# aubin-tchoi/shot-fpfh

Hardware: AMD Instinct MI355X
Metric: descriptors/sec (SHOT+FPFH) on 1M-pt cloud (higher is better)
Workload: dtype f64

## Files before the change

shot_fpfh_amd/csrc/common.h:

```cpp
#pragma once
#include <hip/hip_runtime.h>

#include <cstdarg>
#include <cstdint>
#include <cstdio>
#include <cstring>
#include <map>
#include <atomic>
#include <tuple>
#include <string>
#include <vector>

#include "../../include/shotfpfh.h"

extern std::atomic<unsigned long long> g_sf_sync_count;
static inline hipError_t sf_counted_stream_sync(hipStream_t s)
{
    g_sf_sync_count.fetch_add(1, std::memory_order_relaxed);
    return hipStreamSynchronize(s);
}
#define hipStreamSynchronize(s) sf_counted_stream_sync(s)

#define SF_WAVE 64

// ... 82 lines not shown
    {
        const int rc = sf_palloc(ctx, out, count);
        if (rc == SF_OK) held.push_back((void *)*out);
        return rc;
    }
    void release(void *p)
    {
        for (auto &h : held)
            if (h == p) { sf_pool_release(ctx, p); h = nullptr; }
    }
    ~sf_pool_guard()
    {
        for (void *p : held)
            if (p) sf_pool_release(ctx, p);
    }
};

int sf_comm_allreduce_max_i32(sf_ctx *ctx, const int *send, int *recv, size_t n);
int sf_ctx_scratch(sf_ctx *ctx, size_t bytes, void **out);
#define SF_FLAG_ROWS_GATHER 1
#define SF_FLAG_VOXEL_ORDER 2
int sf_ctx_check_flag(sf_ctx *ctx);
#define SF_PINNED_BYTES 32768
int sf_ctx_pinned(sf_ctx *ctx, void **out);
hipEvent_t sf_ctx_event(sf_ctx *ctx);

struct sf_launch_timer {
    sf_ctx *ctx;
    const char *name;
    hipEvent_t e0 = nullptr, e1 = nullptr;
    bool active;
    sf_launch_timer(sf_ctx *c, const char *n)
        : ctx(c), name(n), active(c->profiling && (c->prof_only.empty() || c->prof_only == n))
    {
        if (active) {
            e0 = sf_ctx_event(ctx);
            e1 = sf_ctx_event(ctx);
            (void)hipEventRecord(e0, ctx->stream);
        }
    }
    ~sf_launch_timer()
    {
        if (active) {
            (void)hipEventRecord(e1, ctx->stream);
            sf_prof_entry &p = ctx->prof[name];
            p.launches++;
            p.pending.emplace_back(e0, e1);
        } else {
            ctx->prof[name].launches++;
        }
    }
};

#define SF_LAUNCH(ctx, name, kernel, grid, block, ...)                                   \
    do {                                                                                 \
        sf_launch_timer t_((ctx), (name));                                               \
        hipLaunchKernelGGL(kernel, (grid), (block), 0, (ctx)->stream, __VA_ARGS__);      \
    } while (0);                                                                         \
    SF_HIP(hipGetLastError())

struct sf_cloud {
    int64_t n = 0;
    double *xyz_orig = nullptr;
    double *nrm_orig = nullptr;
    int32_t *zperm = nullptr;
    int32_t *perm_int = nullptr;
    bool bbox_known = false;
    double bbox_lo[3] = {0, 0, 0}, bbox_hi[3] = {0, 0, 0};
    uint64_t grid_gen = 0;
    double cell = 0.0;
    double inv_cell = 0.0;
    double lo[3] = {0, 0, 0};
    int dim[3] = {1, 1, 1};
    int xsub = 1;
    int64_t ncell = 0;
    int32_t *cell_start = nullptr;
    int32_t *perm = nullptr;
    int32_t *inv_perm = nullptr;
    bool inv_perm_valid = false;
    double *xs = nullptr, *ys = nullptr, *zs = nullptr;
    double *rec = nullptr;
    bool normals_sorted = false;
    double nrm_max2 = -1.0;
    int64_t pop_begin = 0, pop_end = 0;
    double *z_orig = nullptr;
    std::vector<double> z_host;
    int32_t *cell_count = nullptr;
    int64_t cell_count_cap = 0;
    bool count_dirty = false;
    std::vector<int64_t> layer_first;
    std::map<std::pair<double, bool>, std::pair<double, int64_t>> list_stats;
    struct search_record {
        int64_t total = 0, n_overflow = 0, ovf_total = 0, cap = 0, hist[5] = {0, 0, 0, 0, 0};
        int32_t max_count = 0, max_count_all = 0;
        bool folded = false;
    };
    typedef std::tuple<double, double, int, int64_t, int64_t> search_key;
    std::map<search_key, search_record> search_records;
};

struct sf_nbrs {
    int64_t m = 0;
    double radius = 0.0;
    int64_t total = 0;
    int64_t max_count = 0;
    int64_t max_count_all = 0;
    bool view = false;
    bool self = false;
    int64_t self_begin = 0;
    double *qx = nullptr, *qy = nullptr, *qz = nullptr;
    int32_t *qrow = nullptr;
    int32_t *count = nullptr;
    int64_t *offset = nullptr;
    int32_t *idx = nullptr;
    int32_t *idx_ovf = nullptr;
    int64_t cap = 0;
    int64_t n_overflow = 0;
    int64_t hist[5] = {0, 0, 0, 0, 0};
    bool planned = false;
    int main_chunks = 4;
    int tail_limit = 0x7fffffff;
    int32_t *tail_sel = nullptr;
    int64_t n_tail = 0;
    int32_t *mid_sel = nullptr;
    int64_t n_mid = 0;
    int64_t view_first = 0;
    uint64_t grid_gen = 0;
};

static inline void sf_nbrs_stamp(sf_nbrs *nb, const sf_cloud *c) { nb->grid_gen = c->grid_gen; }
static inline int sf_nbrs_on_grid(const sf_nbrs *nb, const sf_cloud *c, const char *who)
{
    if (nb->grid_gen == c->grid_gen) return SF_OK;
    sf_set_error("%s: the neighbour lists were made on another grid of this cloud (build %llu, now %llu): a search with another "
                 "radius, a k-NN search or sf_cloud_build_grid rebuilt it -- search again, or use the lists before the next rebuild",
                 who, (unsigned long long)nb->grid_gen, (unsigned long long)c->grid_gen);
    return SF_ERR_STATE;
}

struct sf_spfh {
    int64_t n = 0;
    int64_t rows_alloc = 0;
    int n_bins = 0;
    int nb3 = 0;
    int stride = 0;
    int elem_bytes = 2;
    int bias = 0;
    int win_lo = 0;
    int win_len = 0;
    void *counts = nullptr;
    int32_t *k = nullptr;
    double *p4 = nullptr;
    unsigned *live = nullptr;
    uint8_t *packed = nullptr;
    uint8_t *hi = nullptr;
    unsigned host_live[2] = {0xffu, ~0u};
    bool host_live_valid = false;
    bool mask_known = false;
};

static inline int64_t sf_div_up(int64_t a, int64_t b) { return (a + b - 1) / b; }

struct sf_dispatch {
    int chunks = 4;
    int limit = 0x7fffffff;
    int tail_limit = 0x7fffffff;
    const int32_t *tail_sel = nullptr;
    int64_t n_tail = 0, view_first = 0;
    const int32_t *mid_sel = nullptr;
    int64_t n_mid = 0;
};
static inline sf_dispatch sf_nbrs_dispatch(const sf_nbrs *nb)
{
    sf_dispatch d;
    if (nb->planned) {
        d.chunks = nb->main_chunks;
        d.limit = nb->n_mid ? 64 * nb->main_chunks : nb->tail_limit;
        d.tail_limit = nb->tail_limit;
        d.tail_sel = nb->tail_sel;
        d.n_tail = nb->n_tail;
        d.mid_sel = nb->mid_sel;
        d.n_mid = nb->n_mid;
        d.view_first = nb->view_first;
    } else {
        const int64_t mx = nb->max_count > 0 ? nb->max_count : 1;
        d.chunks = mx <= 256 ? (int)sf_div_up(mx, 64) : 0;
    }
    return d;
}
```

shot_fpfh_amd/csrc/spfh.hip:

```cpp
#include <algorithm>
#include <cmath>
#include <cstring>

#include "common.h"
#include "device_util.h"

namespace {

#define SF_WIN_FPFH_BINS 11
struct fpfh_edges {
    double a[SF_WIN_FPFH_BINS + 1], p[SF_WIN_FPFH_BINS + 1], t[SF_WIN_FPFH_BINS + 1];
    double tan_t[SF_WIN_FPFH_BINS + 1];
    double p_inv_width;
};

__device__ inline int hist_bin(const double *e, int nb, double x)
{
    if (!(x >= e[0]) || x > e[nb]) return -1;
    int b = 0;
#pragma unroll
    for (int i = 1; i < SF_WIN_FPFH_BINS; ++i)
        if (i < nb && x >= e[i]) b = i;
    return b;
}

__device__ inline int theta_bin(const fpfh_edges &ed, int nb, double a, double b)
{
    const double band = 1e-13;
    const double aa = fabs(a);
    if (b > band * aa) {
        int bin = 0;
        double gap = 1.0e300;
#pragma unroll
        for (int i = 1; i < SF_WIN_FPFH_BINS; ++i)
            if (i < nb) {
                const double di = __builtin_fma(-ed.tan_t[i], b, a);
                bin += di >= 0.0 ? 1 : 0;
                gap = fmin(gap, fabs(di));
            }
        if (gap > band * (aa + fabs(ed.tan_t[1]) * b)) return bin;
    } else if (b < -band * aa) {
        return -1;
    }
    return hist_bin(ed.t, nb, atan2(a, b));
}

__device__ inline int theta_bin_fast(const fpfh_edges &ed, int nb, double a, double b, double E)
{
    const double band = 1e-13;
    const double aa = fabs(a) + E;
    if (b > band * aa) {
        int bin = 0;
        double gap = 1.0e300;
#pragma unroll
        for (int i = 1; i < SF_WIN_FPFH_BINS; ++i)
            if (i < nb) {
                const double di = __builtin_fma(-ed.tan_t[i], b, a);
                bin += di >= 0.0 ? 1 : 0;
                gap = fmin(gap, fabs(di));
            }
        return gap > band * (aa + fabs(ed.tan_t[1]) * b) + E ? bin : -2;
    }
    return b < -band * aa ? -1 : -2;
}

#ifndef SF_SPFH_WPB
#define SF_SPFH_WPB 2
#endif

template <typename CT, int NCH, int NB, bool SEL>
__global__ __launch_bounds__(64 * SF_SPFH_WPB) __attribute__((amdgpu_waves_per_eu((NCH == 0 || NCH >= 4) ? 5 : 6))) void k_spfh(const double *__restrict__ rec,
                                              const int64_t *__restrict__ offset, const int32_t *__restrict__ cnt,
    const int32_t *__restrict__ idx,
                                              int64_t m, int64_t self_begin, fpfh_edges ed, int nb_rt, int nb3, int stride,
                                              CT *__restrict__ counts, int32_t *__restrict__ kout, unsigned bias,
                                              double *__restrict__ p4, double mom_radius, double *__restrict__ cov,
                                              unsigned *__restrict__ live, int alpha_bin, double nrm_max,
                                              uint8_t *__restrict__ packed, int pack_b0, int pack_b1,
                                              uint8_t *__restrict__ hi, int limit, const int32_t *__restrict__ sel,
                                              int64_t nsel, int64_t view_first, int alpha_pair, int win_lo, int win_len)
{
    const int nb = NB > 0 ? NB : nb_rt;
    __shared__ unsigned int hist[SF_SPFH_WPB][SF_FAST_FPFH_BINS * SF_FAST_FPFH_BINS * SF_FAST_FPFH_BINS];
    const int lane = threadIdx.x & 63, wave = threadIdx.x >> 6;
    int64_t q = sf_uniform64(sf_xcd_block() * SF_SPFH_WPB + wave);
    if (SEL) {
        if (q >= nsel) return;
        q = (int64_t)sf_uniform(sel[q]) - view_first;
        if (q < 0) return;
    }
    if (q >= m) return;
    unsigned int *h = hist[wave];
    for (int b = lane; b < win_len; b += 64) h[b] = 0;
    const int64_t i = self_begin + q;
    const int64_t s = offset[q];
    const int k = cnt[q];
#ifndef SF_AB_NOLIMIT
    if (!SEL && sf_uniform(k) > limit) return;
#endif
    const double px = rec[6 * i + 0], py = rec[6 * i + 1], pz = rec[6 * i + 2];
    const double ux = rec[6 * i + 3], uy = rec[6 * i + 4], uz = rec[6 * i + 5];
    __builtin_amdgcn_wave_barrier();
    const double p_inv_width = ed.p_inv_width;
    const double uu = (ux * ux + uy * uy) + uz * uz;
    const double e_per_dist = 1.5e-14 * nrm_max * uu;
    auto pair = [&](double cx, double cy, double cz, double njx, double njy, double njz) {
        const double d2 = (cx * cx + cy * cy) + cz * cz;
        if (d2 > 0.0) {
            const double num = (cx * ux + cy * uy) + cz * uz;
            const double y0 = __builtin_amdgcn_rsq(d2);
            const double y1 = __builtin_fma(0.5 * y0, __builtin_fma(-(d2 * y0), y0, 1.0), y0);
            double phi = num * y1;
            const double pos = (phi - ed.p[0]) * p_inv_width;
            if (fabs(pos - rint(pos)) <= 1e-9) phi = num / sqrt(d2);
            const double b = (njx * ux + njy * uy) + __builtin_fma(njz, uz, 0.0);
            constexpr bool EVEN = NB > 0 && NB % 2 == 0;
            int ba = alpha_bin, bt = -2;
            if (alpha_bin >= 0 || (EVEN && alpha_pair >= 0)) {
                const double nc = (njx * cx + njy * cy) + njz * cz;
                bt = theta_bin_fast(ed, nb, nc * uu - b * num, b, e_per_dist * (d2 * y1) * 1.01);
            }
            if (!EVEN) {
                if (bt == -2) {
                    const double vx = cy * uz - cz * uy, vy = cz * ux - cx * uz, vz = cx * uy - cy * ux;
                    if (alpha_bin < 0) ba = hist_bin(ed.a, nb, (vx * njx + vz * njz) + vy * njy);
                    const double wx = uy * vz - uz * vy, wy = uz * vx - ux * vz, wz = ux * vy - uy * vx;
                    bt = theta_bin(ed, nb, (njx * wx + njz * wz) + njy * wy, b);
                }
            } else if (bt == -2 || alpha_bin < 0) {
                const double vx = cy * uz - cz * uy, vy = cz * ux - cx * uz, vz = cx * uy - cy * ux;
                if (bt == -2) {
                    const double wx = uy * vz - uz * vy, wy = uz * vx - ux * vz, wz = ux * vy - uy * vx;
                    bt = theta_bin(ed, nb, (njx * wx + njz * wz) + njy * wy, b);
                }
                if (alpha_bin < 0) {
                    const double alpha = (vx * njx + vz * njz) + vy * njy;
                    ba = alpha_pair >= 0 ? alpha_pair + (alpha >= ed.a[alpha_pair + 1] ? 1 : 0) : hist_bin(ed.a, nb, alpha);
                }
            }
            const int bp = hist_bin(ed.p, nb, phi);
            if ((ba | bp | bt) >= 0) atomicAdd(&h[(ba * nb + bp) * nb + bt - win_lo], 1u);
        }
    };
    double ws = 0, a11 = 0, a21 = 0, a31 = 0, a22 = 0, a32 = 0, a33 = 0;
    auto moments = [&](double cx, double cy, double cz) {
        const double w = mom_radius - sf_sqrt_fast((cx * cx + cy * cy) + cz * cz);
        ws += w;
        const double wx = cx * w, wy = cy * w, wz = cz * w;
        a11 = __builtin_fma(cx, wx, a11); a21 = __builtin_fma(cy, wx, a21); a31 = __builtin_fma(cz, wx, a31);
        a22 = __builtin_fma(cy, wy, a22); a32 = __builtin_fma(cz, wy, a32); a33 = __builtin_fma(cz, wz, a33);
    };
    if (NCH > 0) {
        constexpr int NC = NCH > 0 ? NCH : 1;
        const int ku = sf_uniform(k);
        int jj[NC];
#pragma unroll
        for (int c = 0; c < NC; ++c) {
            const int t = c * 64 + lane;
            jj[c] = -1;
            if (c == 0 || c * 64 < ku) jj[c] = t < k ? SF_LIST_LOAD(idx + s + t) : -1;
        }
        double cx[NC], cy[NC], cz[NC], ax[NC], ay[NC], az[NC];
#pragma unroll
        for (int c = 0; c < NC; ++c) {
            cx[c] = cy[c] = cz[c] = ax[c] = ay[c] = az[c] = 0.0;
            if (c == 0 || c * 64 < ku) {
                const int j = jj[c] < 0 ? 0 : jj[c];
                sf_load_pn(rec, j, cx[c], cy[c], cz[c], ax[c], ay[c], az[c]);
            }
        }
#pragma unroll
        for (int c = 0; c < NC; ++c)
            if ((c == 0 || c * 64 < ku) && jj[c] >= 0) {
                if (cov) moments(cx[c] - px, cy[c] - py, cz[c] - pz);
                pair(cx[c] - px, cy[c] - py, cz[c] - pz, ax[c], ay[c], az[c]);
            }
    } else {
        for (int t = lane; t < k; t += 64) {
            double x, y, z, a, b, c;
            sf_load_pn(rec, idx[s + t], x, y, z, a, b, c);
            if (cov) moments(x - px, y - py, z - pz);
            pair(x - px, y - py, z - pz, a, b, c);
        }
    }
    if (cov) {
        const double part[8] = {ws, a11, a21, a31, a22, a32, a33, 0.0};
        const double tot = sf_wave_sum8(part);
        const double wsum = __hiloint2double(__builtin_amdgcn_readlane(__double2hiint(tot), 0),
                                             __builtin_amdgcn_readlane(__double2loint(tot), 0));
        const double iw = sf_rcp_fast(wsum);
        const int e = lane >> 3;
        if ((lane & 7) == 0 && e >= 1 && e <= 6) cov[6 * q + e - 1] = tot * iw;
    }
    __builtin_amdgcn_wave_barrier();
    __threadfence_block();
    CT *row = counts + i * (int64_t)stride;
    bool hi_empty = false;
    if (live) {
        const unsigned v0 = lane < win_len ? h[lane] : 0u, v1 = lane + 64 < win_len ? h[lane + 64] : 0u;
        __builtin_nontemporal_store((CT)(v0 ^ bias), row + lane);
        __builtin_nontemporal_store((CT)(v1 ^ bias), row + lane + 64);
        if (hi && sf_uniform(k) > 255) {
            hi[i * 128 + lane] = (uint8_t)(v0 >> 8);
            hi[i * 128 + lane + 64] = (uint8_t)(v1 >> 8);
            hi_empty = __ballot(((v0 | v1) >> 8) != 0u) == 0ull;
        }
        if (packed && lane < 8) {
            const int first = 16 * (lane < 4 ? pack_b0 : pack_b1) + 4 * (lane & 3);
            unsigned w = 0u;
#pragma unroll
            for (int t = 0; t < 4; ++t) w |= (((first + t < win_len ? h[first + t] : 0u) ^ bias) & 0xffu) << (8 * t);
            reinterpret_cast<unsigned *>(packed + i * 32)[lane] = w;
        }
        const unsigned long long n0 = __ballot(v0 != 0u), n1 = __ballot(v1 != 0u);
        unsigned mask = 0u;
#pragma unroll
        for (int kq = 0; kq < 4; ++kq) {
            mask |= ((n0 >> (16 * kq)) & 0xffffull) ? 1u << kq : 0u;
            mask |= ((n1 >> (16 * kq)) & 0xffffull) ? 16u << kq : 0u;
        }
        if (lane == 0 && (mask & ~*live)) atomicOr(live, mask);
    } else {
        for (int b = lane; b < stride; b += 64) row[b] = (CT)((b < nb3 ? h[b] : 0u) ^ bias);
    }
    if (lane == 0) {
        kout[i] = k;
        if (p4) {
            double2 *o = reinterpret_cast<double2 *>(p4 + 4 * i);
            o[0] = make_double2(rec[6 * i + 0], rec[6 * i + 1]);
            o[1] = make_double2(rec[6 * i + 2], hi_empty ? -(double)k : (double)k);
        }
    }
}

__device__ inline void spfh_pack_row(const uint8_t *__restrict__ counts, uint8_t *__restrict__ packed, int64_t row, unsigned mask)
{
    const int b0 = mask ? __ffs(mask) - 1 : 0;
    const unsigned rest = mask & (mask - 1u);
    const int b1 = rest ? __ffs(rest) - 1 : (b0 + 1) & 7;
    const uint4 *src = reinterpret_cast<const uint4 *>(counts + row * 128);
    uint4 *dst = reinterpret_cast<uint4 *>(packed + row * 32);
    dst[0] = src[b0];
    dst[1] = src[b1];
}

__global__ __launch_bounds__(256) void k_spfh_pack(const uint8_t *__restrict__ counts, int64_t begin, int64_t end,
                                                   const unsigned *__restrict__ live, uint8_t *__restrict__ packed)
{
    const unsigned mask = live[0] & 0xffu;
    if (__popc(mask) > 2) return;
    const int64_t row = begin + (int64_t)blockIdx.x * blockDim.x + threadIdx.x;
    if (row < end) spfh_pack_row(counts, packed, row, mask);
}

__global__ __launch_bounds__(256) void k_spfh_repack(const uint8_t *__restrict__ counts, int64_t n, int64_t begin, int64_t end,
                                                     const unsigned *__restrict__ live, uint8_t *__restrict__ packed)
{
    const unsigned mask = live[0] & 0xffu, sig = live[1];
    if (__popc(mask) > 2 || sig == mask) return;
    for (int64_t row = (int64_t)blockIdx.x * blockDim.x + threadIdx.x; row < n; row += (int64_t)gridDim.x * blockDim.x)
        if (row < begin || row >= end) spfh_pack_row(counts, packed, row, mask);
}

__global__ void k_spfh_live_or(unsigned *__restrict__ live, unsigned det) { live[0] |= det; }

__global__ void k_spfh_pack_done(unsigned *__restrict__ live)
{
    const unsigned mask = live[0] & 0xffu;
    live[1] = __popc(mask) <= 2 ? mask : ~0u;
}

template <typename CT>
__global__ void k_spfh_export(const CT *__restrict__ counts, const int32_t *__restrict__ kk,
                              const int32_t *__restrict__ perm, int64_t n, int nb3, int stride, unsigned bias,
                              double *__restrict__ out, const uint8_t *__restrict__ hi, int win_lo, int win_len)
{
    int64_t g = (int64_t)blockIdx.x * blockDim.x + threadIdx.x;
    if (g >= n * nb3) return;
    int64_t i = g / nb3;
    int b = (int)(g - i * nb3);
    const int col = b - win_lo;
    unsigned cnt = 0u;
    if (col >= 0 && col < win_len) {
        cnt = (unsigned)counts[i * stride + col] ^ bias;
        if (hi && kk[i] > 255) cnt += 256u * (unsigned)hi[i * stride + col];
    }
    out[(int64_t)perm[i] * nb3 + b] = (double)cnt / (double)kk[i];
}

__device__ inline int hist_bin_search(const double *__restrict__ e, int nb, double x)
{
    if (!(x >= e[0]) || x > e[nb]) return -1;
    if (x == e[nb]) return nb - 1;
    int lo = 0, hi = nb + 1;
    while (lo < hi) {
        const int mid = (lo + hi) >> 1;
        if (e[mid] <= x) lo = mid + 1; else hi = mid;
    }
    return lo - 1;
}

__global__ __launch_bounds__(256) void k_spfh_generic(const double *__restrict__ rec, const int64_t *__restrict__ offset,
                                                      const int32_t *__restrict__ cnt, const int32_t *__restrict__ idx, int64_t m,
                                                      int64_t self_begin, const double *__restrict__ edges, int nb, int nb3,
                                                      int stride, unsigned *__restrict__ counts, int32_t *__restrict__ kk)
{
    const int lane = threadIdx.x & 63;
    const int64_t q = sf_uniform64(sf_xcd_block() * 4 + (threadIdx.x >> 6));
    if (q >= m) return;
    const int64_t i = self_begin + q, s = offset[q];
    const int k = cnt[q];
    unsigned *row = counts + i * (int64_t)stride;
    for (int b = lane; b < stride; b += 64) row[b] = 0u;
    if (lane == 0) kk[i] = k;
    __threadfence();
    double px, py, pz, ux, uy, uz;
    sf_load_pn(rec, (int)i, px, py, pz, ux, uy, uz);
    const double *ea = edges, *ep = edges + (nb + 1), *et = edges + 2 * (nb + 1);
    for (int t = lane; t < k; t += 64) {
        double x, y, z, nx, ny, nz;
        sf_load_pn(rec, idx[s + t], x, y, z, nx, ny, nz);
        const double cx = x - px, cy = y - py, cz = z - pz;
        const double dist = sqrt((cx * cx + cy * cy) + cz * cz);
        if (!(dist > 0.0)) continue;
        const double vx = cy * uz - cz * uy, vy = cz * ux - cx * uz, vz = cx * uy - cy * ux;
        const double wx = uy * vz - uz * vy, wy = uz * vx - ux * vz, wz = ux * vy - uy * vx;
        const double alpha = (vx * nx + vz * nz) + vy * ny;
        const double phi = (((cx * ux + cy * uy) + cz * uz) + 0.0) / dist;
        const double theta = atan2((nx * wx + nz * wz) + ny * wy, ((nx * ux + ny * uy) + nz * uz) + 0.0);
        const int ba = hist_bin_search(ea, nb, alpha), bp = hist_bin_search(ep, nb, phi), bt = hist_bin_search(et, nb, theta);
        if (ba < 0 || bp < 0 || bt < 0) continue;
        atomicAdd(&row[(ba * nb + bp) * nb + bt], 1u);
    }
}
}


static bool alpha_bins_within_reach(const double *edges_a, int nb, double reach, int *first, int *last)
{
    if (!(reach >= 0.0) || !std::isfinite(reach) || !(-reach > edges_a[0]) || !(reach < edges_a[nb])) return false;
    int lo = 0, hi = 0;
    for (int i = 1; i < nb; ++i) {
        if (edges_a[i] <= -reach) lo = i;
        if (edges_a[i] <= reach) hi = i;
    }
    *first = lo;
    *last = hi;
    return true;
}

static sf_spfh *spfh_create(sf_ctx *ctx, sf_cloud *c, int n_bins, int64_t max_count, double radius);

extern "C" sf_spfh *sf_spfh_create(sf_ctx *ctx, sf_cloud *c, int n_bins, int64_t max_count)
{
    return spfh_create(ctx, c, n_bins, max_count, 0.0);
}

extern "C" sf_spfh *sf_spfh_create_for_radius(sf_ctx *ctx, sf_cloud *c, int n_bins, int64_t max_count, double radius)
{
    return spfh_create(ctx, c, n_bins, max_count, radius);
}

extern "C" int sf_spfh_elem_bytes(const sf_spfh *sp) { return sp ? sp->elem_bytes : 0; }

static sf_spfh *spfh_create(sf_ctx *ctx, sf_cloud *c, int n_bins, int64_t max_count, double radius)
{
    if (!ctx || !c) { sf_set_error("sf_spfh_create: null argument"); return nullptr; }
    if (n_bins < 1 || n_bins > SF_MAX_FPFH_BINS) {
        sf_set_error("sf_spfh_create: n_bins=%d outside 1..%d (n_bins^3 bins per point)", n_bins, SF_MAX_FPFH_BINS);
        return nullptr;
    }
    if (hipSetDevice(ctx->device) != hipSuccess) { sf_set_error("hipSetDevice failed"); return nullptr; }
    sf_spfh *sp = new sf_spfh();
    sp->n = c->n;
    sp->n_bins = n_bins;
    sp->nb3 = n_bins * n_bins * n_bins;
    sp->win_lo = 0;
    sp->win_len = sp->nb3;
    bool window = false;
    if (sp->nb3 > 128 && n_bins <= SF_WIN_FPFH_BINS && max_count <= 65535 && radius > 0.0 && c->nrm_orig && !getenv("SF_FPFH_NO_WINDOW")) {
        double n2 = 0.0, ea[SF_WIN_FPFH_BINS + 1];
        if (sf_cloud_normals_max2(ctx, c, &n2) != SF_OK) { delete sp; return nullptr; }
        for (int i = 0; i <= n_bins; ++i) ea[i] = -1.0 + 2.0 * (double)i / (double)n_bins;
        int a0 = 0, a1 = 0;
        if (alpha_bins_within_reach(ea, n_bins, radius * n2 * (1.0 + 1e-6), &a0, &a1) && (a1 - a0 + 1) * n_bins * n_bins <= 128) {
            window = true;
            sp->win_lo = a0 * n_bins * n_bins;
            sp->win_len = (a1 - a0 + 1) * n_bins * n_bins;
        }
    }
    sp->elem_bytes = (max_count <= 65535 && (sp->nb3 <= 128 || window)) ? 1 : (max_count > 65535 ? 4 : 2);
    if (n_bins > SF_FAST_FPFH_BINS && !window) sp->elem_bytes = 4;
    sp->bias = sp->elem_bytes == 1 ? 128 : 0;
    sp->stride = 128;
    while (sp->stride < (window ? sp->win_len : sp->nb3)) sp->stride *= 2;
    if (n_bins > SF_FAST_FPFH_BINS && !window) sp->stride = (sp->nb3 + 3) & ~3;
    const int64_t nr = ctx->nranks > 0 ? ctx->nranks : 1;
    sp->rows_alloc = std::max<int64_t>(sf_div_up(c->n, nr) * nr, 1);
    size_t nn = (size_t)sp->rows_alloc;
    if ((double)nn * sp->stride * sp->elem_bytes > 2.0e11) {
        sf_set_error("sf_spfh_create: an SPFH table of %lld x %d bins does not fit the device", (long long)nn, sp->nb3);
        delete sp;
        return nullptr;
    }
    const bool bytes_tab = sp->elem_bytes == 1;
    bool ok = sf_pool_alloc(ctx, nn * sp->stride * sp->elem_bytes, &sp->counts) == SF_OK && sf_pool_alloc(ctx, nn * sizeof(int32_t), (void **)&sp->k) == SF_OK;
    if (ok && bytes_tab) ok = sf_pool_alloc(ctx, nn * 4 * sizeof(double), (void **)&sp->p4) == SF_OK;
    if (ok && bytes_tab && max_count > 255) ok = sf_pool_alloc(ctx, nn * 128, (void **)&sp->hi) == SF_OK;
    if (ok && bytes_tab)
        ok = sf_pool_alloc(ctx, 4 * sizeof(unsigned), (void **)&sp->live) == SF_OK && sf_pool_alloc(ctx, nn * 32, (void **)&sp->packed) == SF_OK &&
             hipMemsetAsync(sp->live, 0, 4 * sizeof(unsigned), ctx->stream) == hipSuccess &&
             hipMemsetAsync(sp->live, getenv("SF_FPFH_DENSE") ? 0xff : 0, sizeof(unsigned), ctx->stream) == hipSuccess &&
             hipMemsetAsync(sp->live + 1, 0xff, sizeof(unsigned), ctx->stream) == hipSuccess;
    if (!ok) {
        sf_set_error("sf_spfh_create: out of device memory");
        sf_spfh_free(ctx, sp);
        return nullptr;
    }
    sp->host_live[0] = getenv("SF_FPFH_DENSE") ? ~0u : 0u;
    sp->host_live[1] = ~0u;
    sp->host_live_valid = sp->mask_known = sp->elem_bytes == 1;
    return sp;
}

extern "C" void sf_spfh_free(sf_ctx *ctx, sf_spfh *sp)
{
    if (!sp) return;
    if (ctx) (void)hipStreamSynchronize(ctx->stream);
    for (void *p : {(void *)sp->counts, (void *)sp->k, (void *)sp->p4, (void *)sp->live, (void *)sp->packed, (void *)sp->hi})
        if (p) { if (ctx) sf_pool_release(ctx, p); else (void)hipFree(p); }
    delete sp;
}

static int spfh_compute(sf_ctx *ctx, sf_cloud *c, sf_nbrs *nb, sf_spfh *sp, const double *edges, double *cov)
{
    if (!ctx || !c || !nb || !sp || !edges) { sf_set_error("sf_spfh_compute: null argument"); return SF_ERR_ARG; }
    if (!nb->self) { sf_set_error("sf_spfh_compute: needs a sf_radius_search_self result"); return SF_ERR_ARG; }
    SF_CHECK(sf_nbrs_on_grid(nb, c, "sf_spfh_compute"));
    if (sp->n != c->n || nb->self_begin + nb->m > sp->n) { sf_set_error("sf_spfh_compute: table/cloud size mismatch"); return SF_ERR_ARG; }
    if (sp->elem_bytes == 1 && nb->max_count > 255 && !sp->hi) {
        sf_set_error("sf_spfh_compute: neighbourhood of %lld points needs a wider table (pass max_count to sf_spfh_create)",
                     (long long)nb->max_count);
        return SF_ERR_ARG;
    }
    if (sp->elem_bytes <= 2 && nb->max_count > 65535) {
        sf_set_error("sf_spfh_compute: neighbourhood of %lld points needs a 32-bit table (pass max_count to sf_spfh_create)",
                     (long long)nb->max_count);
        return SF_ERR_ARG;
    }
    SF_HIP(hipSetDevice(ctx->device));
    SF_CHECK(sf_cloud_ensure_sorted_normals(ctx, c));
    if (sp->n_bins > SF_FAST_FPFH_BINS && sp->elem_bytes != 1) {
        if (cov) { sf_set_error("sf_spfh_compute_moments: n_bins=%d has no shared-sweep form (use sf_spfh_compute)", sp->n_bins); return SF_ERR_UNSUPPORTED; }
        const int64_t mg = nb->m;
        if (!mg) return SF_OK;
        sf_pool_guard tmp(ctx);
        double *dedges = nullptr;
        const size_t ne = (size_t)3 * (sp->n_bins + 1);
        SF_CHECK(tmp.alloc(&dedges, ne));
        SF_HIP(hipMemcpyAsync(dedges, edges, ne * sizeof(double), hipMemcpyHostToDevice, ctx->stream));
        SF_LAUNCH(ctx, "k6_spfh", k_spfh_generic, dim3(sf_xcd_grid(sf_div_up(mg, 4))), dim3(256), c->rec, nb->offset, nb->count,
                  nb->idx, mg, nb->self_begin, (const double *)dedges, sp->n_bins, sp->nb3, sp->stride, (unsigned *)sp->counts, sp->k);
        SF_HIP(hipStreamSynchronize(ctx->stream));
        return SF_OK;
    }
    fpfh_edges ed;
    const int nbn = sp->n_bins;
    for (int i = 0; i <= SF_WIN_FPFH_BINS; ++i) {
        ed.a[i] = edges[i <= nbn ? i : nbn];
        ed.p[i] = edges[(nbn + 1) + (i <= nbn ? i : nbn)];
        ed.t[i] = edges[2 * (nbn + 1) + (i <= nbn ? i : nbn)];
        ed.tan_t[i] = std::tan(ed.t[i]);
    }
    ed.p_inv_width = (double)nbn / (ed.p[nbn] - ed.p[0]);
    const int64_t m = nb->m;
    if (!m) return SF_OK;
    int alpha_bin = -1, alpha_pair = -1;
    double nrm_max = 1.0;
    {
        double n2 = 0.0;
        SF_CHECK(sf_cloud_normals_max2(ctx, c, &n2));
        nrm_max = std::sqrt(n2) * (1.0 + 1e-12);
        const double reach = nb->radius * n2 * (1.0 + 1e-9);
        double nearest = INFINITY;
        for (int i = 0; i <= nbn; ++i) nearest = std::min(nearest, std::fabs(ed.a[i]));
        if (std::isfinite(reach) && reach < nearest)
            for (int i = 0; i < nbn; ++i)
                if (ed.a[i] < 0.0 && 0.0 < ed.a[i + 1]) alpha_bin = i;
        int a0 = 0, a1 = 0;
        const bool within = alpha_bins_within_reach(ed.a, nbn, reach, &a0, &a1);
        if (alpha_bin < 0 && within && a1 == a0 + 1) alpha_pair = a0;
        if (getenv("SF_FPFH_NO_ALPHA_SHORTCUT")) alpha_bin = alpha_pair = -1;
        if (sp->elem_bytes == 1 && sp->win_len != sp->nb3) {
            if (!within || a0 * nbn * nbn < sp->win_lo || (a1 + 1) * nbn * nbn > sp->win_lo + sp->win_len) {
                sf_set_error("sf_spfh_compute: the table keeps bins %d .. %d of %d (created for a smaller radius); a search radius of %g "
                             "reaches other alpha bins -- create the table for this radius", sp->win_lo, sp->win_lo + sp->win_len - 1,
                             sp->nb3, nb->radius);
                return SF_ERR_STATE;
            }
        }
    }
    const dim3 grid(sf_xcd_grid(sf_div_up(m, SF_SPFH_WPB))), block(64 * SF_SPFH_WPB);
    const sf_dispatch dsp = sf_nbrs_dispatch(nb);
    const dim3 grid_tail(sf_xcd_grid(sf_div_up(dsp.n_tail > 0 ? dsp.n_tail : 1, SF_SPFH_WPB)));
    const dim3 grid_mid(sf_xcd_grid(sf_div_up(dsp.n_mid > 0 ? dsp.n_mid : 1, SF_SPFH_WPB)));
    uint8_t *const hi_rows = sp->elem_bytes == 1 ? sp->hi : nullptr;
#define SF_SPFH_NB(NAME, GRID, CT, NCH, NB, SEL, SELP, NSEL)                                                            \
    SF_LAUNCH(ctx, NAME, (k_spfh<CT, NCH, NB, SEL>), GRID, block, c->rec, nb->offset, nb->count, nb->idx, m,            \
              nb->self_begin, ed, nbn, sp->nb3, sp->stride, (CT *)sp->counts, sp->k, (unsigned)sp->bias, sp->p4, nb->radius, cov, \
              sizeof(CT) == 1 ? sp->live : (unsigned *)nullptr, alpha_bin, nrm_max, fused_packed, fused_b0, fused_b1,   \
              hi_rows, dsp.limit, SELP, NSEL, dsp.view_first, alpha_pair, sizeof(CT) == 1 ? sp->win_lo : 0,                \
              sizeof(CT) == 1 ? sp->win_len : sp->nb3)
#define SF_SPFH_WIDE_1(NAME, GRID, CT, NCH, SEL, SELP, NSEL)                                                            \
    if (nbn == 9) { SF_SPFH_NB(NAME, GRID, CT, NCH, 9, SEL, SELP, NSEL); }                                              \
    else if (nbn == 11) { SF_SPFH_NB(NAME, GRID, CT, NCH, 11, SEL, SELP, NSEL); }                                       \
    else { sf_set_error("sf_spfh_compute: no fast kernel for %d bins", nbn); return SF_ERR_UNSUPPORTED; }
#define SF_SPFH_WIDE_0(NAME, GRID, CT, NCH, SEL, SELP, NSEL)                                                            \
    { sf_set_error("sf_spfh_compute: no fast kernel for %d bins on this table", nbn); return SF_ERR_UNSUPPORTED; }
#define SF_SPFH_LAUNCH(NAME, GRID, CT, NCH, SEL, SELP, NSEL, WIDE)                                                            \
    switch (nbn) {                    \
    case 1: { SF_SPFH_NB(NAME, GRID, CT, NCH, 1, SEL, SELP, NSEL); } break;                                            \
    case 2: { SF_SPFH_NB(NAME, GRID, CT, NCH, 2, SEL, SELP, NSEL); } break;                                            \
    case 3: { SF_SPFH_NB(NAME, GRID, CT, NCH, 3, SEL, SELP, NSEL); } break;                                            \
    case 4: { SF_SPFH_NB(NAME, GRID, CT, NCH, 4, SEL, SELP, NSEL); } break;                                            \
    case 5: { SF_SPFH_NB(NAME, GRID, CT, NCH, 5, SEL, SELP, NSEL); } break;                                            \
    case 6: { SF_SPFH_NB(NAME, GRID, CT, NCH, 6, SEL, SELP, NSEL); } break;                                            \
    case 7: { SF_SPFH_NB(NAME, GRID, CT, NCH, 7, SEL, SELP, NSEL); } break;                                            \
    case 8: { SF_SPFH_NB(NAME, GRID, CT, NCH, 8, SEL, SELP, NSEL); } break;                                            \
    default: { SF_SPFH_WIDE_##WIDE(NAME, GRID, CT, NCH, SEL, SELP, NSEL); } break;                                       \
    }
#define SF_SPFH_DISPATCH(CT, WIDE)                                                                        \
    switch (dsp.chunks) {                                                                           \
    case 1: { SF_SPFH_LAUNCH("k6_spfh", grid, CT, 1, false, (const int32_t *)nullptr, (int64_t)0, WIDE); } break;                \
    case 2: { SF_SPFH_LAUNCH("k6_spfh", grid, CT, 2, false, (const int32_t *)nullptr, (int64_t)0, WIDE); } break;                \
    case 3: { SF_SPFH_LAUNCH("k6_spfh", grid, CT, 3, false, (const int32_t *)nullptr, (int64_t)0, WIDE); } break;                \
    case 4: { SF_SPFH_LAUNCH("k6_spfh", grid, CT, 4, false, (const int32_t *)nullptr, (int64_t)0, WIDE); } break;                \
    default: { SF_SPFH_LAUNCH("k6_spfh", grid, CT, 0, false, (const int32_t *)nullptr, (int64_t)0, WIDE); } break;               \
    }                                                                                               \
    if (dsp.n_mid) { SF_SPFH_LAUNCH("k6_spfh_mid", grid_mid, CT, 4, true, dsp.mid_sel, dsp.n_mid, WIDE); } \
    if (dsp.n_tail) { SF_SPFH_LAUNCH("k6_spfh_tail", grid_tail, CT, 0, true, dsp.tail_sel, dsp.n_tail, WIDE); }
    uint8_t *fused_packed = nullptr;
    int fused_b0 = -1, fused_b1 = -1;
    if (sp->elem_bytes == 1) {
        unsigned det = 0u;
        const int pin0 = alpha_bin >= 0 ? alpha_bin : alpha_pair, pin1 = alpha_bin >= 0 ? alpha_bin : alpha_pair + 1;
        if (pin0 >= 0)
            for (int blk = (pin0 * nbn * nbn - sp->win_lo) / 16; blk <= ((pin1 + 1) * nbn * nbn - 1 - sp->win_lo) / 16; ++blk) det |= 1u << blk;
        const unsigned m8 = sp->host_live[0] & 0xffu;
        if (det && sp->mask_known && sp->host_live_valid && (m8 | det) == m8 && __builtin_popcount(m8) <= 2 && sp->host_live[1] == m8) {
            fused_packed = sp->packed;
            fused_b0 = m8 ? __builtin_ffs((int)m8) - 1 : 0;
            const unsigned rest = m8 & (m8 - 1u);
            fused_b1 = rest ? __builtin_ffs((int)rest) - 1 : (fused_b0 + 1) & 7;
            SF_SPFH_DISPATCH(uint8_t, 1)
            return SF_OK;
        }
        if (det) SF_LAUNCH(ctx, "k6_spfh_pack", k_spfh_live_or, dim3(1), dim3(1), sp->live, det);
        SF_SPFH_DISPATCH(uint8_t, 1)
        SF_LAUNCH(ctx, "k6_spfh_pack", k_spfh_pack, dim3((unsigned)sf_div_up(m, 256)), dim3(256), (const uint8_t *)sp->counts,
                  nb->self_begin, nb->self_begin + m, (const unsigned *)sp->live, sp->packed);
        SF_LAUNCH(ctx, "k6_spfh_pack", k_spfh_repack, dim3(2048), dim3(256), (const uint8_t *)sp->counts, sp->n, nb->self_begin,
                  nb->self_begin + m, (const unsigned *)sp->live, sp->packed);
        SF_LAUNCH(ctx, "k6_spfh_pack", k_spfh_pack_done, dim3(1), dim3(1), sp->live);
        if (det && sp->mask_known) {
            sp->host_live[0] |= det;
            const unsigned m8 = sp->host_live[0] & 0xffu;
            sp->host_live[1] = __builtin_popcount(m8) <= 2 ? m8 : ~0u;
            sp->host_live_valid = true;
        } else {
            sp->mask_known = false;
            sp->host_live_valid = false;
        }
    } else if (sp->elem_bytes == 2) {
        SF_SPFH_DISPATCH(uint16_t, 0)
    } else {
        SF_SPFH_DISPATCH(uint32_t, 0)
    }
#undef SF_SPFH_DISPATCH
#undef SF_SPFH_WIDE_1
#undef SF_SPFH_WIDE_0
#undef SF_SPFH_LAUNCH
#undef SF_SPFH_NB
    return SF_OK;
}

extern "C" int sf_spfh_compute(sf_ctx *ctx, sf_cloud *c, sf_nbrs *nb, sf_spfh *sp, const double *edges)
{
    return spfh_compute(ctx, c, nb, sp, edges, nullptr);
}

extern "C" int sf_spfh_compute_moments(sf_ctx *ctx, sf_cloud *c, sf_nbrs *nb, sf_spfh *sp, const double *edges,
                                       double *cov_dev)
{
    if (!cov_dev) { sf_set_error("sf_spfh_compute_moments: null cov"); return SF_ERR_ARG; }
    return spfh_compute(ctx, c, nb, sp, edges, cov_dev);
}

extern "C" int sf_spfh_allgather(sf_ctx *ctx, sf_spfh *sp, int64_t rows_per_rank)
{
    if (!ctx || !sp) { sf_set_error("sf_spfh_allgather: null argument"); return SF_ERR_ARG; }
    if (ctx->nranks == 1 && !ctx->comm) return SF_OK;
    if (rows_per_rank <= 0 || rows_per_rank * ctx->nranks > sp->rows_alloc || rows_per_rank * ctx->nranks < sp->n) {
        sf_set_error("sf_spfh_allgather: %lld rows/rank x %d ranks does not tile a table of %lld (+pad %lld) rows",
                     (long long)rows_per_rank, ctx->nranks, (long long)sp->n, (long long)sp->rows_alloc);
        return SF_ERR_ARG;
    }
    const size_t row_bytes = (size_t)sp->stride * sp->elem_bytes;
    char *base = (char *)sp->counts;
    if (ctx->comm && ctx->nranks > 1) {
        sf_pool_guard tmp(ctx);
        int *fw = nullptr;
        SF_CHECK(tmp.alloc(&fw, 2));
        const int word = (int)sp->elem_bytes | (sp->hi ? 1 << 8 : 0) | (sp->p4 ? 1 << 9 : 0) | ((int)sp->stride << 12);
        void *pin = nullptr;
        SF_CHECK(sf_ctx_pinned(ctx, &pin));
        int *hw = (int *)((char *)pin + SF_PINNED_BYTES - 16);
        hw[0] = word;
        hw[1] = -word;
        SF_HIP(hipMemcpyAsync(fw, hw, 2 * sizeof(int), hipMemcpyHostToDevice, ctx->stream));
        SF_CHECK(sf_comm_allreduce_max_i32(ctx, fw, fw, 2));
        SF_HIP(hipMemcpyAsync(hw, fw, 2 * sizeof(int), hipMemcpyDeviceToHost, ctx->stream));
        SF_HIP(hipStreamSynchronize(ctx->stream));
        if (hw[0] != word || hw[1] != -word) {
            sf_set_error("sf_spfh_allgather: the ranks hold SPFH tables of different storage (this rank: %d-byte counts%s%s, stride %d; "
                         "format words over the ranks %#x .. %#x) -- size every rank's table by the longest list of ANY rank",
                         sp->elem_bytes, sp->hi ? " + high-byte rows" : "", sp->p4 ? " + packed rows" : "", (int)sp->stride,
                         (unsigned)-hw[1], (unsigned)hw[0]);
            return SF_ERR_STATE;
        }
    }
    SF_CHECK(sf_comm_allgather(ctx, base + (size_t)ctx->rank * rows_per_rank * row_bytes, base,
                               (size_t)rows_per_rank * row_bytes));
    char *kb = (char *)sp->k;
    SF_CHECK(sf_comm_allgather(ctx, kb + (size_t)ctx->rank * rows_per_rank * sizeof(int32_t), kb,
                               (size_t)rows_per_rank * sizeof(int32_t)));
    if (sp->p4) {
        char *pb = (char *)sp->p4;
        SF_CHECK(sf_comm_allgather(ctx, pb + (size_t)ctx->rank * rows_per_rank * 32, pb, (size_t)rows_per_rank * 32));
    }
    if (sp->hi) {
        char *hb = (char *)sp->hi;
        SF_CHECK(sf_comm_allgather(ctx, hb + (size_t)ctx->rank * rows_per_rank * 128, hb, (size_t)rows_per_rank * 128));
    }
    if (sp->live) {
        SF_HIP(hipMemsetAsync(sp->live, 0xff, 2 * sizeof(unsigned), ctx->stream));
        sp->host_live[0] = sp->host_live[1] = ~0u;
        sp->host_live_valid = sp->mask_known = true;
    }
    return SF_OK;
}

struct spfh_part { char *base; size_t row; };
#define SF_WIRE_PARTS 3
static int spfh_wire_parts(sf_ctx *ctx, sf_spfh *sp, spfh_part parts[SF_WIRE_PARTS])
{
    parts[2] = spfh_part{nullptr, 0};
    if (sp->elem_bytes == 1) {
        const unsigned m8 = sp->host_live[0] & 0xffu;
        const bool sparse = sp->mask_known && sp->host_live_valid && __builtin_popcount(m8) <= 2 && sp->host_live[1] == m8;
        if (!sparse) {
            SF_HIP(hipMemsetAsync(sp->live, 0xff, 2 * sizeof(unsigned), ctx->streams[0]));
            sp->host_live[0] = sp->host_live[1] = ~0u;
            sp->host_live_valid = sp->mask_known = true;
        }
        parts[0] = sparse ? spfh_part{(char *)sp->packed, 32} : spfh_part{(char *)sp->counts, 128};
// ... 97 lines not shown
```

Before: 564.1 million.

## Add symmetric theta binning, direct phi bin, DPP wave sum, and edge-exact theta

For odd bin counts with symmetric theta edges, the fast theta bin compares |a| against only the upper half of the tangents and mirrors the result by sign. The phi bin now comes from the already computed position instead of a separate edge search, falling back to the search only near edges or out of range. The moment reduction uses a permlane/DPP-based wave sum, and the histogram clear and readout drop bounds checks for the byte table. Theta bins near edges are also resolved with extended-precision boundary tangents, and profiling markers compiled out by default are added. The extra edge tables and precision fallback code raise register use and complexity.

```diff
diff --git a/shot_fpfh_amd/csrc/common.h b/shot_fpfh_amd/csrc/common.h
--- a/shot_fpfh_amd/csrc/common.h
+++ b/shot_fpfh_amd/csrc/common.h
@@ -258,6 +258,9 @@
     int32_t *k = nullptr;
     double *p4 = nullptr;
     unsigned *live = nullptr;
+    double *theta_m = nullptr;
+    double theta_m_host[36] = {0};
+    bool theta_m_valid = false;
     uint8_t *packed = nullptr;
     uint8_t *hi = nullptr;
     unsigned host_live[2] = {0xffu, ~0u};
diff --git a/shot_fpfh_amd/csrc/spfh.hip b/shot_fpfh_amd/csrc/spfh.hip
--- a/shot_fpfh_amd/csrc/spfh.hip
+++ b/shot_fpfh_amd/csrc/spfh.hip
@@ -1,6 +1,7 @@
 #include <algorithm>
 #include <cmath>
 #include <cstring>
+#include <vector>
 
 #include "common.h"
 #include "device_util.h"
@@ -24,7 +25,16 @@
     return b;
 }
 
-__device__ inline int theta_bin(const fpfh_edges &ed, int nb, double a, double b)
+__device__ inline double theta_at_edge(double t, double a, double b, double e, const double *__restrict__ tm, int i, int stride)
+{
+    if (e == 0.0 || !(fabs(t - e) <= 1e-15 * fabs(e))) return t;
+    const double tm_hi = tm[i], tm_lo = tm[stride + i];
+    const double d = __builtin_fma(-tm_lo, b, __builtin_fma(-tm_hi, b, a));
+    if (!(fabs(d) > 1e-18 * (fabs(a) + fabs(tm_hi * b)))) return t;
+    return d >= 0.0 ? e : e - 2e-15 * fabs(e);
+}
+
+__device__ inline int theta_bin(const fpfh_edges &ed, int nb, double a, double b, const double *__restrict__ tm)
 {
     const double band = 1e-13;
     const double aa = fabs(a);
@@ -38,13 +48,29 @@
                 bin += di >= 0.0 ? 1 : 0;
                 gap = fmin(gap, fabs(di));
             }
-        if (gap > band * (aa + fabs(ed.tan_t[1]) * b)) return bin;
+        const double near = band * (aa + fabs(ed.tan_t[1]) * b);
+        if (gap > near) return bin;
+        bool decided = true;
+        bin = 0;
+#pragma unroll 1
+        for (int i = 1; i < nb; ++i) {
+            const double di = __builtin_fma(-tm[2 * (SF_WIN_FPFH_BINS + 1) + i], b, a);
+            double d = di;
+            if (!(fabs(di) > near)) {
+                const double hi = tm[i];
+                d = __builtin_fma(-tm[SF_WIN_FPFH_BINS + 1 + i], b, __builtin_fma(-hi, b, a));
+                if (hi == 0.0 || !(fabs(d) > 1e-18 * (aa + fabs(hi * b)))) decided = false;
+            }
+            bin += d >= 0.0 ? 1 : 0;
+        }
+        if (decided) return bin;
     } else if (b < -band * aa) {
         return -1;
     }
     return hist_bin(ed.t, nb, atan2(a, b));
 }
 
+template <bool SYM>
 __device__ inline int theta_bin_fast(const fpfh_edges &ed, int nb, double a, double b, double E)
 {
     const double band = 1e-13;
@@ -52,6 +78,20 @@
     if (b > band * aa) {
         int bin = 0;
         double gap = 1.0e300;
+        if (SYM) {
+            const int mid = (nb - 1) >> 1;
+            const double fa = fabs(a);
+#pragma unroll
+            for (int j = 1; j < SF_WIN_FPFH_BINS; ++j)
+                if (j < nb && j > mid) {
+                    const double dj = __builtin_fma(-ed.tan_t[j], b, fa);
+                    bin += dj >= 0.0 ? 1 : 0;
+                    gap = fmin(gap, fabs(dj));
+                }
+            const int sgn = __double2hiint(a) >> 31;
+            bin = mid + ((bin ^ sgn) - sgn);
+            return gap > band * (aa + ed.tan_t[nb - 1] * b) + E ? bin : -2;
+        }
 #pragma unroll
         for (int i = 1; i < SF_WIN_FPFH_BINS; ++i)
             if (i < nb) {
@@ -62,6 +102,59 @@
         return gap > band * (aa + fabs(ed.tan_t[1]) * b) + E ? bin : -2;
     }
     return b < -band * aa ? -1 : -2;
+}
+
+#ifdef SF_K6_MARK_BUILD
+#define SF_K6_MARK(id)                                                          \
+    do {                                                                        \
+        __builtin_amdgcn_sched_barrier(0);                                      \
+        asm volatile("; K6MARK %0" ::"n"(id));                                  \
+        __builtin_amdgcn_sched_barrier(0);                                      \
+    } while (0)
+#define SF_K6_PIN(x) asm volatile("" : "+v"(x))
+#else
+#define SF_K6_MARK(id) do { } while (0)
+#define SF_K6_PIN(x) (void)(x)
+#endif
+
+__device__ inline double spfh_swap_add(double keep_lo, double keep_hi, bool half)
+{
+    const unsigned al = (unsigned)__double2loint(keep_lo), ah = (unsigned)__double2hiint(keep_lo);
+    const unsigned bl = (unsigned)__double2loint(keep_hi), bh = (unsigned)__double2hiint(keep_hi);
+    if (half) {
+        const auto l = __builtin_amdgcn_permlane32_swap(al, bl, false, false), h = __builtin_amdgcn_permlane32_swap(ah, bh, false, false);
+        return __hiloint2double((int)h[0], (int)l[0]) + __hiloint2double((int)h[1], (int)l[1]);
+    }
+    const auto l = __builtin_amdgcn_permlane16_swap(al, bl, false, false), h = __builtin_amdgcn_permlane16_swap(ah, bh, false, false);
+    return __hiloint2double((int)h[0], (int)l[0]) + __hiloint2double((int)h[1], (int)l[1]);
+}
+
+__device__ inline double spfh_wave_sum8(const double (&v)[8])
+{
+    const bool b3 = sf_lane() & 8;
+    double k4[4], k2[2];
+#pragma unroll
+    for (int i = 0; i < 4; ++i) k4[i] = spfh_swap_add(v[i], v[4 + i], true);
+#pragma unroll
+    for (int i = 0; i < 2; ++i) k2[i] = spfh_swap_add(k4[i], k4[2 + i], false);
+    double r;
+    {
+        const double mine = b3 ? k2[1] : k2[0], send = b3 ? k2[0] : k2[1];
+        const int lo = __builtin_amdgcn_update_dpp(0, __double2loint(send), 0x128, 0xf, 0xf, true);
+        const int hi = __builtin_amdgcn_update_dpp(0, __double2hiint(send), 0x128, 0xf, 0xf, true);
+        r = mine + __hiloint2double(hi, lo);
+    }
+#define SF_DPP_ADD(ctrl)                                                                                  \
+    {                                                                                                     \
+        const int lo = __builtin_amdgcn_update_dpp(0, __double2loint(r), ctrl, 0xf, 0xf, true);          \
+        const int hi = __builtin_amdgcn_update_dpp(0, __double2hiint(r), ctrl, 0xf, 0xf, true);          \
+        r += __hiloint2double(hi, lo);                                                                    \
+    }
+    SF_DPP_ADD(0xB1)
+    SF_DPP_ADD(0x4E)
+    SF_DPP_ADD(0x141)
+#undef SF_DPP_ADD
+    return r;
 }
 
 #ifndef SF_SPFH_WPB
@@ -78,7 +171,8 @@
                                               unsigned *__restrict__ live, int alpha_bin, double nrm_max,
                                               uint8_t *__restrict__ packed, int pack_b0, int pack_b1,
                                               uint8_t *__restrict__ hi, int limit, const int32_t *__restrict__ sel,
-                                              int64_t nsel, int64_t view_first, int alpha_pair, int win_lo, int win_len)
+                                              int64_t nsel, int64_t view_first, int alpha_pair, int win_lo, int win_len, int theta_sym,
+                                              const double *__restrict__ theta_m)
 {
     const int nb = NB > 0 ? NB : nb_rt;
     __shared__ unsigned int hist[SF_SPFH_WPB][SF_FAST_FPFH_BINS * SF_FAST_FPFH_BINS * SF_FAST_FPFH_BINS];
@@ -90,8 +184,10 @@
         if (q < 0) return;
     }
     if (q >= m) return;
+    SF_K6_MARK(1);
     unsigned int *h = hist[wave];
-    for (int b = lane; b < win_len; b += 64) h[b] = 0;
+    if (sizeof(CT) == 1) h[lane] = h[lane + 64] = 0;
+    else for (int b = lane; b < win_len; b += 64) h[b] = 0;
     const int64_t i = self_begin + q;
     const int64_t s = offset[q];
     const int k = cnt[q];
@@ -105,6 +201,7 @@
     const double uu = (ux * ux + uy * uy) + uz * uz;
     const double e_per_dist = 1.5e-14 * nrm_max * uu;
     auto pair = [&](double cx, double cy, double cz, double njx, double njy, double njz) {
+        SF_K6_MARK(31);
         const double d2 = (cx * cx + cy * cy) + cz * cz;
         if (d2 > 0.0) {
             const double num = (cx * ux + cy * uy) + cz * uz;
@@ -112,38 +209,65 @@
             const double y1 = __builtin_fma(0.5 * y0, __builtin_fma(-(d2 * y0), y0, 1.0), y0);
             double phi = num * y1;
             const double pos = (phi - ed.p[0]) * p_inv_width;
-            if (fabs(pos - rint(pos)) <= 1e-9) phi = num / sqrt(d2);
+            int bp;
+#ifndef SF_SPFH_NO_PHI_POS
+            const bool near_edge = fabs(pos - rint(pos)) <= 1e-9;
+            if (near_edge || !(pos > 0.0) || !(pos < (double)nb)) {
+                SF_K6_MARK(39);
+                if (near_edge) phi = num / sqrt(d2);
+                bp = hist_bin(ed.p, nb, phi);
+            } else {
+                bp = (int)pos;
+            }
+#else
+            if (fabs(pos - rint(pos)) <= 1e-9) { SF_K6_MARK(39); phi = num / sqrt(d2); }
+            bp = hist_bin(ed.p, nb, phi);
+#endif
+            SF_K6_PIN(bp);
+            SF_K6_MARK(32);
             const double b = (njx * ux + njy * uy) + __builtin_fma(njz, uz, 0.0);
             constexpr bool EVEN = NB > 0 && NB % 2 == 0;
             int ba = alpha_bin, bt = -2;
             if (alpha_bin >= 0 || (EVEN && alpha_pair >= 0)) {
                 const double nc = (njx * cx + njy * cy) + njz * cz;
-                bt = theta_bin_fast(ed, nb, nc * uu - b * num, b, e_per_dist * (d2 * y1) * 1.01);
+                const double a_fast = nc * uu - b * num, e_fast = e_per_dist * (d2 * y1) * 1.01;
+                if (NB > 2 && NB % 2 == 1 && theta_sym) {
+                    bt = theta_bin_fast<true>(ed, nb, a_fast, b, e_fast);
+                } else {
+                    SF_K6_MARK(38);
+                    bt = theta_bin_fast<false>(ed, nb, a_fast, b, e_fast);
+                }
+                SF_K6_PIN(bt);
+                SF_K6_MARK(32);
             }
             if (!EVEN) {
                 if (bt == -2) {
+                    SF_K6_MARK(39);
                     const double vx = cy * uz - cz * uy, vy = cz * ux - cx * uz, vz = cx * uy - cy * ux;
                     if (alpha_bin < 0) ba = hist_bin(ed.a, nb, (vx * njx + vz * njz) + vy * njy);
                     const double wx = uy * vz - uz * vy, wy = uz * vx - ux * vz, wz = ux * vy - uy * vx;
-                    bt = theta_bin(ed, nb, (njx * wx + njz * wz) + njy * wy, b);
+                    bt = theta_bin(ed, nb, (njx * wx + njz * wz) + njy * wy, b, theta_m);
                 }
             } else if (bt == -2 || alpha_bin < 0) {
+                SF_K6_MARK(39);
                 const double vx = cy * uz - cz * uy, vy = cz * ux - cx * uz, vz = cx * uy - cy * ux;
                 if (bt == -2) {
                     const double wx = uy * vz - uz * vy, wy = uz * vx - ux * vz, wz = ux * vy - uy * vx;
-                    bt = theta_bin(ed, nb, (njx * wx + njz * wz) + njy * wy, b);
+                    bt = theta_bin(ed, nb, (njx * wx + njz * wz) + njy * wy, b, theta_m);
                 }
                 if (alpha_bin < 0) {
                     const double alpha = (vx * njx + vz * njz) + vy * njy;
                     ba = alpha_pair >= 0 ? alpha_pair + (alpha >= ed.a[alpha_pair + 1] ? 1 : 0) : hist_bin(ed.a, nb, alpha);
                 }
             }
-            const int bp = hist_bin(ed.p, nb, phi);
+            SF_K6_PIN(bt);
+            SF_K6_MARK(33);
             if ((ba | bp | bt) >= 0) atomicAdd(&h[(ba * nb + bp) * nb + bt - win_lo], 1u);
         }
     };
     double ws = 0, a11 = 0, a21 = 0, a31 = 0, a22 = 0, a32 = 0, a33 = 0;
     auto moments = [&](double cx, double cy, double cz) {
+        SF_K6_MARK(30);
         const double w = mom_radius - sf_sqrt_fast((cx * cx + cy * cy) + cz * cz);
         ws += w;
         const double wx = cx * w, wy = cy * w, wz = cz * w;
@@ -153,6 +277,7 @@
     if (NCH > 0) {
         constexpr int NC = NCH > 0 ? NCH : 1;
         const int ku = sf_uniform(k);
+        SF_K6_MARK(2);
         int jj[NC];
 #pragma unroll
         for (int c = 0; c < NC; ++c) {
@@ -176,6 +301,7 @@
                 pair(cx[c] - px, cy[c] - py, cz[c] - pz, ax[c], ay[c], az[c]);
             }
     } else {
+        SF_K6_MARK(2);
         for (int t = lane; t < k; t += 64) {
             double x, y, z, a, b, c;
             sf_load_pn(rec, idx[s + t], x, y, z, a, b, c);
@@ -183,9 +309,10 @@
             pair(x - px, y - py, z - pz, a, b, c);
         }
     }
+    SF_K6_MARK(4);
     if (cov) {
         const double part[8] = {ws, a11, a21, a31, a22, a32, a33, 0.0};
-        const double tot = sf_wave_sum8(part);
+        const double tot = spfh_wave_sum8(part);
         const double wsum = __hiloint2double(__builtin_amdgcn_readlane(__double2hiint(tot), 0),
                                              __builtin_amdgcn_readlane(__double2loint(tot), 0));
         const double iw = sf_rcp_fast(wsum);
@@ -194,10 +321,11 @@
     }
     __builtin_amdgcn_wave_barrier();
     __threadfence_block();
+    SF_K6_MARK(5);
     CT *row = counts + i * (int64_t)stride;
     bool hi_empty = false;
     if (live) {
-        const unsigned v0 = lane < win_len ? h[lane] : 0u, v1 = lane + 64 < win_len ? h[lane + 64] : 0u;
+        const unsigned v0 = h[lane], v1 = h[lane + 64];
         __builtin_nontemporal_store((CT)(v0 ^ bias), row + lane);
         __builtin_nontemporal_store((CT)(v1 ^ bias), row + lane + 64);
         if (hi && sf_uniform(k) > 255) {
@@ -205,13 +333,15 @@
             hi[i * 128 + lane + 64] = (uint8_t)(v1 >> 8);
             hi_empty = __ballot(((v0 | v1) >> 8) != 0u) == 0ull;
         }
+        SF_K6_MARK(6);
         if (packed && lane < 8) {
             const int first = 16 * (lane < 4 ? pack_b0 : pack_b1) + 4 * (lane & 3);
             unsigned w = 0u;
 #pragma unroll
-            for (int t = 0; t < 4; ++t) w |= (((first + t < win_len ? h[first + t] : 0u) ^ bias) & 0xffu) << (8 * t);
+            for (int t = 0; t < 4; ++t) w |= ((h[first + t] ^ bias) & 0xffu) << (8 * t);
             reinterpret_cast<unsigned *>(packed + i * 32)[lane] = w;
         }
+        SF_K6_MARK(7);
         const unsigned long long n0 = __ballot(v0 != 0u), n1 = __ballot(v1 != 0u);
         unsigned mask = 0u;
 #pragma unroll
@@ -223,12 +353,13 @@
     } else {
         for (int b = lane; b < stride; b += 64) row[b] = (CT)((b < nb3 ? h[b] : 0u) ^ bias);
     }
+    SF_K6_MARK(8);
     if (lane == 0) {
         kout[i] = k;
         if (p4) {
             double2 *o = reinterpret_cast<double2 *>(p4 + 4 * i);
-            o[0] = make_double2(rec[6 * i + 0], rec[6 * i + 1]);
-            o[1] = make_double2(rec[6 * i + 2], hi_empty ? -(double)k : (double)k);
+            o[0] = make_double2(px, py);
+            o[1] = make_double2(pz, hi_empty ? -(double)k : (double)k);
         }
     }
 }
@@ -327,8 +458,16 @@
         const double wx = uy * vz - uz * vy, wy = uz * vx - ux * vz, wz = ux * vy - uy * vx;
         const double alpha = (vx * nx + vz * nz) + vy * ny;
         const double phi = (((cx * ux + cy * uy) + cz * uz) + 0.0) / dist;
-        const double theta = atan2((nx * wx + nz * wz) + ny * wy, ((nx * ux + ny * uy) + nz * uz) + 0.0);
-        const int ba = hist_bin_search(ea, nb, alpha), bp = hist_bin_search(ep, nb, phi), bt = hist_bin_search(et, nb, theta);
+        const double ta = (nx * wx + nz * wz) + ny * wy, tb = ((nx * ux + ny * uy) + nz * uz) + 0.0;
+        double theta = atan2(ta, tb);
+        int bt = hist_bin_search(et, nb, theta);
+        if (bt >= 0) {
+            const double *tm = edges + 3 * (nb + 1);
+            if (bt >= 1) theta = theta_at_edge(theta, ta, tb, et[bt], tm, bt, nb + 1);
+            if (bt + 1 < nb) theta = theta_at_edge(theta, ta, tb, et[bt + 1], tm, bt + 1, nb + 1);
+            bt = hist_bin_search(et, nb, theta);
+        }
+        const int ba = hist_bin_search(ea, nb, alpha), bp = hist_bin_search(ep, nb, phi);
         if (ba < 0 || bp < 0 || bt < 0) continue;
         atomicAdd(&row[(ba * nb + bp) * nb + bt], 1u);
     }
@@ -347,6 +486,24 @@
     *first = lo;
     *last = hi;
     return true;
+}
+
+static bool theta_edges_symmetric(const double *tan_t, int nb)
+{
+    if (nb < 3 || nb % 2 == 0) return false;
+    for (int j = (nb - 1) / 2 + 1; j < nb; ++j) {
+        const double lo = -tan_t[nb - j];
+        if (!(tan_t[j] > 0.0) || !std::isfinite(tan_t[j]) || std::memcmp(&tan_t[j], &lo, sizeof(double)) != 0) return false;
+    }
+    return true;
+}
+
+static void theta_boundary_tan(double e, double *hi, double *lo)
+{
+    const long double m = ((long double)e + (long double)std::nextafter(e, -INFINITY)) / 2.0L;
+    const long double t = tanl(m);
+    *hi = (double)t;
+    *lo = (double)(t - (long double)*hi);
 }
 
 static sf_spfh *spfh_create(sf_ctx *ctx, sf_cloud *c, int n_bins, int64_t max_count, double radius);
@@ -405,6 +562,7 @@
     }
     const bool bytes_tab = sp->elem_bytes == 1;
     bool ok = sf_pool_alloc(ctx, nn * sp->stride * sp->elem_bytes, &sp->counts) == SF_OK && sf_pool_alloc(ctx, nn * sizeof(int32_t), (void **)&sp->k) == SF_OK;
+    if (ok) ok = sf_pool_alloc(ctx, 3 * (SF_WIN_FPFH_BINS + 1) * sizeof(double), (void **)&sp->theta_m) == SF_OK;
     if (ok && bytes_tab) ok = sf_pool_alloc(ctx, nn * 4 * sizeof(double), (void **)&sp->p4) == SF_OK;
     if (ok && bytes_tab && max_count > 255) ok = sf_pool_alloc(ctx, nn * 128, (void **)&sp->hi) == SF_OK;
     if (ok && bytes_tab)
@@ -427,7 +585,7 @@
 {
     if (!sp) return;
     if (ctx) (void)hipStreamSynchronize(ctx->stream);
-    for (void *p : {(void *)sp->counts, (void *)sp->k, (void *)sp->p4, (void *)sp->live, (void *)sp->packed, (void *)sp->hi})
+    for (void *p : {(void *)sp->counts, (void *)sp->k, (void *)sp->p4, (void *)sp->live, (void *)sp->packed, (void *)sp->hi, (void *)sp->theta_m})
         if (p) { if (ctx) sf_pool_release(ctx, p); else (void)hipFree(p); }
     delete sp;
 }
@@ -456,9 +614,13 @@
         if (!mg) return SF_OK;
         sf_pool_guard tmp(ctx);
         double *dedges = nullptr;
-        const size_t ne = (size_t)3 * (sp->n_bins + 1);
+        const size_t ne1 = (size_t)sp->n_bins + 1, ne = 5 * ne1;
         SF_CHECK(tmp.alloc(&dedges, ne));
-        SF_HIP(hipMemcpyAsync(dedges, edges, ne * sizeof(double), hipMemcpyHostToDevice, ctx->stream));
+        std::vector<double> he(ne, 0.0);
+        std::memcpy(he.data(), edges, 3 * ne1 * sizeof(double));
+        for (int i = 1; i < sp->n_bins; ++i)
+            if (edges[2 * ne1 + i] != 0.0) theta_boundary_tan(edges[2 * ne1 + i], &he[3 * ne1 + i], &he[4 * ne1 + i]);
+        SF_HIP(hipMemcpyAsync(dedges, he.data(), ne * sizeof(double), hipMemcpyHostToDevice, ctx->stream));
         SF_LAUNCH(ctx, "k6_spfh", k_spfh_generic, dim3(sf_xcd_grid(sf_div_up(mg, 4))), dim3(256), c->rec, nb->offset, nb->count,
                   nb->idx, mg, nb->self_begin, (const double *)dedges, sp->n_bins, sp->nb3, sp->stride, (unsigned *)sp->counts, sp->k);
         SF_HIP(hipStreamSynchronize(ctx->stream));
@@ -472,7 +634,19 @@
         ed.t[i] = edges[2 * (nbn + 1) + (i <= nbn ? i : nbn)];
         ed.tan_t[i] = std::tan(ed.t[i]);
     }
+    {
+        double tm[3 * (SF_WIN_FPFH_BINS + 1)] = {0};
+        for (int i = 0; i <= SF_WIN_FPFH_BINS; ++i) tm[2 * (SF_WIN_FPFH_BINS + 1) + i] = ed.tan_t[i];
+        for (int i = 1; i < nbn; ++i)
+            if (ed.t[i] != 0.0) theta_boundary_tan(ed.t[i], &tm[i], &tm[SF_WIN_FPFH_BINS + 1 + i]);
+        if (!sp->theta_m_valid || std::memcmp(tm, sp->theta_m_host, sizeof(tm)) != 0) {
+            std::memcpy(sp->theta_m_host, tm, sizeof(tm));
+            SF_HIP(hipMemcpyAsync(sp->theta_m, sp->theta_m_host, sizeof(tm), hipMemcpyHostToDevice, ctx->stream));
+            sp->theta_m_valid = true;
+        }
+    }
     ed.p_inv_width = (double)nbn / (ed.p[nbn] - ed.p[0]);
+    const int theta_sym = theta_edges_symmetric(ed.tan_t, nbn) && !getenv("SF_FPFH_NO_THETA_SYM");
     const int64_t m = nb->m;
     if (!m) return SF_OK;
     int alpha_bin = -1, alpha_pair = -1;
@@ -510,7 +684,7 @@
               nb->self_begin, ed, nbn, sp->nb3, sp->stride, (CT *)sp->counts, sp->k, (unsigned)sp->bias, sp->p4, nb->radius, cov, \
               sizeof(CT) == 1 ? sp->live : (unsigned *)nullptr, alpha_bin, nrm_max, fused_packed, fused_b0, fused_b1,   \
               hi_rows, dsp.limit, SELP, NSEL, dsp.view_first, alpha_pair, sizeof(CT) == 1 ? sp->win_lo : 0,                \
-              sizeof(CT) == 1 ? sp->win_len : sp->nb3)
+              sizeof(CT) == 1 ? sp->win_len : sp->nb3, theta_sym, (const double *)sp->theta_m)
 #define SF_SPFH_WIDE_1(NAME, GRID, CT, NCH, SEL, SELP, NSEL)                                                            \
     if (nbn == 9) { SF_SPFH_NB(NAME, GRID, CT, NCH, 9, SEL, SELP, NSEL); }                                              \
     else if (nbn == 11) { SF_SPFH_NB(NAME, GRID, CT, NCH, 11, SEL, SELP, NSEL); }                                       \
```

New measurement: 573.2 million (median of 6 runs). 1.6% higher.
